# Sovik-Ghosh/SFM

Hardware: AMD Instinct MI355X
Metric: BA LM-iterations/sec + descriptor-pairs/sec, 200 cams / 100k pts, 1->8 MI355X (higher is better)
Workload: dtype f64; 1 GPU; BA: 200 cams / 100000 pts / 1000000 obs, cam block 10 (reference 10-parameter block + regulariser), aligned residual order, Huber, SciPy-TRF control flow, fixed schedule; parallelism=points sharded over 1 rank(s), cameras replicated, RCCL all-reduce of [S|r], comm=single rank, seed=1004

## Files before the change

### sfm_amd/csrc/ba.hip

```cpp
#include "ba_internal.h"
#include <cstdlib>
#include <type_traits>
#include <cmath>
#include <atomic>
#include <chrono>

typedef double v4d __attribute__((ext_vector_type(4)));

__device__ __forceinline__ void publish_word(double* word, double seq) {
  if (seq > 0.0) {
    __threadfence_system();
    *(volatile double*)word = seq;
  }
}
__device__ __forceinline__ void publish_ticket(double* hsc, double seq) { publish_word(hsc + SFM_HSC_SEQ, seq); }

#define EPS_D 2.220446049250313e-16
#define SQRT_EPS_D 1.4901161193847656e-08
#define CAMPRE 16

static int64_t g_stride(int64_t D) { return D == 10 ? 32 : 3 * D; }

Lay ba_layout(int64_t C, int64_t P, int64_t N, int64_t D, int64_t n_items, int64_t n_cchunks, int precision) {
  Lay L;
// ... 916 lines not shown
  }
  __syncthreads();
  if (Einv && r < c_0 + ASM_NB && e < D)
    diag_block_factor_lanes<D>(&sOut[0][(r - c_0) * D], ASM_NB * D + 1, alpha, e, r, Einv, Efac, cg_scal);
  const int n = C * D, W = nv * D;
  constexpr int WMAX = ASM_NB * D, NST = (D * WMAX + 127) / 128;
#pragma unroll
  for (int t = 0; t < NST; ++t) {
    const int idx = e + 128 * t;
    const int rr = idx / WMAX, col = idx - rr * WMAX;
    if (rr < D && col < W) S[(size_t)(r * D + rr) * n + c_0 * D + col] = sOut[rr][col];
  }
}

template <int D>
__global__ __launch_bounds__(128) void k_schur_diag(int C, const int* __restrict__ item_ptr, const double* __restrict__ part,
                                                    const double* __restrict__ B, double alpha, double* __restrict__ Einv,
                                                    double* __restrict__ Efac, double* __restrict__ cg_scal) {
  __shared__ double sBlk[D][D + 1];
  const int r = blockIdx.x, e = threadIdx.x;
  if (e < D * D) {
    const int rr = e / D, col = e - rr * D;
    const int64_t blk = (int64_t)r * C - (int64_t)r * (r - 1) / 2;
    double s = 0.0;
#pragma unroll 4
    for (int it = item_ptr[blk]; it < item_ptr[blk + 1]; ++it) s += part[(size_t)it * (D * D) + e];
    double v = -s;
    v += B[(size_t)r * D * D + e];
    sBlk[rr][col] = v;
  }
  __syncthreads();
  if (e < D) diag_block_factor_lanes<D>(&sBlk[0][0], D + 1, alpha, e, r, Einv, Efac, cg_scal);
}
template <int D, int ASM_NB>
__global__ __launch_bounds__(128) void k_schur_assemble_scaled(int C, const int* __restrict__ item_ptr, const double* __restrict__ part,
                                                               const double* __restrict__ B, double* __restrict__ St,
                                                               const int* __restrict__ cch_ptr, const double* __restrict__ cch_part,
                                                               const double* __restrict__ gc, double* __restrict__ rhs_out,
                                                               double* __restrict__ rhs_t, double alpha, const double* __restrict__ Einv) {
  constexpr int SCALED_BAND = 128 / D + 2;
  if (blockIdx.y == 0 && threadIdx.x < 64) {
    const int cc = blockIdx.x, lane = threadIdx.x, sl = lane >> 4, a = lane & 15;
    double t = 0.0;
    for (int ch = cch_ptr[cc] + sl; ch < cch_ptr[cc + 1]; ch += 4) t += cch_part[(size_t)ch * 16 + a];
    const double t1 = __shfl(t, a + 16, 64), t2 = __shfl(t, a + 32, 64), t3 = __shfl(t, a + 48, 64);
    const double rv = (sl == 0 && a < D) ? gc[cc * D + a] - ((t + t1) + (t2 + t3)) : 0.0;
    double ts = 0.0;
#pragma unroll
    for (int k = 0; k < D; ++k) ts += Einv[(size_t)cc * D * D + (a < D ? a : 0) * D + k] * __shfl(rv, k, 64);
    if (sl == 0 && a < D) { rhs_out[cc * D + a] = rv; rhs_t[cc * D + a] = ts; }
  }
  __shared__ double sOut[D][ASM_NB * D + 1];
  __shared__ double sE1[D * D], sE2[ASM_NB][D * D];
  const int r = blockIdx.x, c_0 = blockIdx.y * ASM_NB;
  if (c_0 > r) return;
  const int nv = (r - c_0 + 1) < ASM_NB ? (r - c_0 + 1) : ASM_NB;
  const int e = threadIdx.x;
  const int a = e / D, b = e - a * D;
  if (e < D * D) {
    double ev[ASM_NB + 1];
    ev[ASM_NB] = Einv[(size_t)r * D * D + e];
#pragma unroll
    for (int j = 0; j < ASM_NB; ++j) ev[j] = j < nv ? Einv[(size_t)(c_0 + j) * D * D + e] : 0.0;
    double v[ASM_NB];
    strip_item_sums<D, ASM_NB>(C, r, c_0, nv, e, item_ptr, part, B, v);
    sE1[e] = ev[ASM_NB];
#pragma unroll
    for (int j = 0; j < ASM_NB; ++j)
      if (j < nv) { sOut[a][j * D + b] = v[j]; sE2[j][e] = ev[j]; }
  }
  __syncthreads();
  const bool has_diag = r < c_0 + ASM_NB;
  const int jd = (r - c_0) * D;
  double dv = 0.0;
  if (has_diag && e < D * D) dv = (b <= a ? sOut[a][jd + b] : sOut[b][jd + a]) + (a == b ? alpha : 0.0);
  __syncthreads();
  if (has_diag && e < D * D) sOut[a][jd + b] = dv;
  __syncthreads();
  constexpr int RPT = 1;
  constexpr int RH = D / RPT;
  const int oj = e / RH, oh = e - oj * RH;
  const bool owner = e < ASM_NB * RH && oj < nv;
  double out[RPT][D];
  if (owner) {
#pragma unroll
    for (int q = 0; q < RPT; ++q) {
      const int ra = oh + q * RH;
      double tr[D];
#pragma unroll
      for (int bb = 0; bb < D; ++bb) tr[bb] = 0.0;
#pragma unroll
      for (int k = 0; k < D; ++k) {
        const double e1 = sE1[ra * D + k];
#pragma unroll
        for (int bb = 0; bb < D; ++bb) tr[bb] = fma(e1, sOut[k][oj * D + bb], tr[bb]);
        __builtin_amdgcn_sched_barrier(0);
      }
#pragma unroll
      for (int bb = 0; bb < D; ++bb) {
        double t = 0.0;
#pragma unroll
        for (int k = 0; k < D; ++k) t = fma(tr[k], sE2[oj][bb * D + k], t);
        out[q][bb] = t;
        __builtin_amdgcn_sched_barrier(0);
      }
    }
  }
  __syncthreads();
  if (owner) {
#pragma unroll
    for (int q = 0; q < RPT; ++q)
#pragma unroll
      for (int bb = 0; bb < D; ++bb) sOut[oh + q * RH][oj * D + bb] = out[q][bb];
  }
  __syncthreads();
  const int n = C * D, W = nv * D;
  constexpr int WMAX = ASM_NB * D, NST = (D * WMAX + 127) / 128;
#pragma unroll
  for (int t = 0; t < NST; ++t) {
    const int idx = e + 128 * t;
    const int rr = idx / WMAX, col = idx - rr * WMAX;
    if (rr < D && col < W) St[(size_t)(r * D + rr) * n + c_0 * D + col] = sOut[rr][col];
  }
  if (e < D * D) {
#pragma unroll
    for (int j = 0; j < ASM_NB; ++j) {
      const int c = c_0 + j;
      if (j < nv && c < r && r - c <= SCALED_BAND)
        St[(size_t)(c * D + a) * n + r * D + b] = sOut[b][j * D + a];
    }
  }
}

template <int D, typename T, int GS>
__global__ __launch_bounds__(256) void k_cam_reduce_chunks(const int* __restrict__ cch_beg, const int* __restrict__ cch_end,
                                                           const int* __restrict__ cam_obs, const int* __restrict__ cam_pt,
                                                           const T* __restrict__ G, const double* __restrict__ vec,
                                                           double* __restrict__ part) {
  static_assert(D % 2 == 0 && GS % 2 == 0 && GS <= 32, "16-byte pieces of a block: one per lane of a 16-lane group");
  typedef T pair_t __attribute__((ext_vector_type(2)));
  __shared__ double s[4][4][32];
  const int ch = blockIdx.x, tid = threadIdx.x, lane = tid & 63, w = tid >> 6;
  const int grp = lane >> 4, l16 = lane & 15;
  const int e0 = 2 * l16;
  const bool live = e0 < 3 * D;
  const int m = live ? e0 / D : 0;
  double acc0 = 0.0, acc1 = 0.0;
  const int beg = cch_beg[ch], end = cch_end[ch];
  constexpr int UNR = 4;
  for (int i0 = beg + w * 4 + grp; i0 < end; i0 += 16 * UNR) {
// ... 1 lines not shown
    pair_t g[UNR];
    double vm[UNR];
#pragma unroll
    for (int u = 0; u < UNR; ++u) { const int i = i0 + 16 * u; k[u] = i < end ? cam_obs[i] : -1; pj[u] = i < end ? cam_pt[i] : 0; }
#pragma unroll
    for (int u = 0; u < UNR; ++u) {
      g[u] = (k[u] >= 0 && live) ? *(const pair_t*)(G + (size_t)k[u] * GS + e0) : (pair_t){(T)0, (T)0};
    }
#pragma unroll
    for (int u = 0; u < UNR; ++u) vm[u] = k[u] >= 0 ? vec[(size_t)pj[u] * 3 + m] : 0.0;
#pragma unroll
    for (int u = 0; u < UNR; ++u)
      if (k[u] >= 0 && live) { acc0 += (double)g[u].x * vm[u]; acc1 += (double)g[u].y * vm[u]; }
  }
  s[w][grp][e0] = acc0; s[w][grp][e0 + 1] = acc1;
  __syncthreads();
  if (tid < 16) {
    double t = 0.0;
    if (tid < D) {
#pragma unroll
      for (int mm = 0; mm < 3; ++mm)
#pragma unroll
        for (int ww = 0; ww < 4; ++ww)
#pragma unroll
          for (int gg = 0; gg < 4; ++gg) t += s[ww][gg][mm * D + tid];
    }
    part[(size_t)ch * 16 + tid] = t;
  }
}
template <int D>
__global__ __launch_bounds__(256) void k_cam_reduce_final(int C, const int* __restrict__ cch_ptr, const double* __restrict__ part,
                                                          const double* __restrict__ base, double* __restrict__ out,
                                                          const double* __restrict__ sum_part = nullptr, int sum_nblk = 0, int sum_cnt = 0,
                                                          double* __restrict__ sum_dst = nullptr) {
  if (sum_part && blockIdx.x == gridDim.x - 1) {
    __shared__ double s_red[4];
    for (int q = 0; q < sum_cnt; ++q) {
      double t = 0.0;
      for (int i = threadIdx.x; i < sum_nblk; i += 256) t += sum_part[(size_t)i * sum_cnt + q];
      const double tt = block_sum256(t, s_red);
      if (threadIdx.x == 0) sum_dst[q] = tt;
    }
    return;
  }
  const int c = blockIdx.x * 4 + (threadIdx.x >> 6);
  if (c >= C) return;
  const int lane = threadIdx.x & 63, s = lane >> 4, a = lane & 15;
  double t = 0.0;
  for (int ch = cch_ptr[c] + s; ch < cch_ptr[c + 1]; ch += 4) t += part[(size_t)ch * 16 + a];
  const double t1 = __shfl(t, a + 16, 64), t2 = __shfl(t, a + 32, 64), t3 = __shfl(t, a + 48, 64);
  if (s == 0 && a < D) out[c * D + a] = (base ? base[c * D + a] : 0.0) - ((t + t1) + (t2 + t3));
}

constexpr int GTP_OBS = 64;
template <int D, typename T, int GS>
__global__ __launch_bounds__(256) void k_obs_Gtp(int64_t N, const int* __restrict__ cam_idx,
                                                 const T* __restrict__ G,
                                                 const double* __restrict__ pc, double* __restrict__ tmp3) {
  static_assert(D % 2 == 0 && GS % 2 == 0 && GS <= 32, "16-byte pieces of a block: one per lane of a 16-lane group");
  typedef T pair_t __attribute__((ext_vector_type(2)));
  __shared__ double s[GTP_OBS][17];
  const int tid = threadIdx.x, slot = tid >> 4, l16 = tid & 15;
  const int64_t k0 = (int64_t)blockIdx.x * GTP_OBS;
  const int e0 = 2 * l16;
  const int a = e0 % D;
  const bool live = e0 < 3 * D;
  pair_t g[GTP_OBS / 16];
  int cam[GTP_OBS / 16];
#pragma unroll
  for (int it = 0; it < GTP_OBS / 16; ++it) {
    const int64_t k = k0 + it * 16 + slot;
    const bool ok = live && k < N;
    g[it] = ok ? *(const pair_t*)(G + (size_t)k * GS + e0) : (pair_t)(T)0;
    cam[it] = ok ? cam_idx[k] : 0;
  }
#pragma unroll
  for (int it = 0; it < GTP_OBS / 16; ++it) {
    const double2 p = *(const double2*)(pc + (size_t)cam[it] * D + a);
    s[it * 16 + slot][l16] = (double)g[it].x * p.x + (double)g[it].y * p.y;
  }
  __syncthreads();
  if (tid < 3 * GTP_OBS) {
    const int sl = tid / 3, mm = tid - 3 * sl;
    const int64_t kk = k0 + sl;
// ... 383 lines not shown
  }
  hipLaunchKernelGGL(k_lin_finalize, dim3(1), dim3(256), 0, h->stream, n, D, WS(L, gc), WS(L, B), WS(L, part_obs),
                     (int)L.nblk_obs, WS(L, part_pt), (int)L.nblk_pt, WS(L, cost_reg), nreg, WS(L, red_lin),
                     WS(L, gmax));
  sfm_prof_end(h, SFM_PROF_LIN_REST);
  SFM_LAUNCH_CHECK(h, "sfm_ba_linearize");
  return SFM_OK;
}

extern "C" int sfm_ba_finish_linearize(sfm_handle h, sfm_ba_problem p) {
  Lay L; int rc = check_problem(h, p, &L); if (rc) return rc;
  double* ws = (double*)p->workspace;
  hipLaunchKernelGGL(k_finish_linearize, dim3(1), dim3(256), 0, h->stream, p->n_cams * p->cam_dim,
                     WS(L, red_lin), WS(L, gmax), WS(L, scalars), p->host_sc, next_ticket(p));
  SFM_LAUNCH_CHECK(h, "sfm_ba_finish_linearize");
  return SFM_OK;
}

static void launch_schur_assemble(sfm_ctx* h, sfm_ba_problem p, const Lay& L, double alpha, double* einv_out, double* m_out) {
  double* ws = (double*)p->workspace;
  const int C = p->n_cams, D = p->cam_dim, n = C * D;
  const AsmShape shape = schur_assemble_shape(C);
#define ASM_LAUNCH(NB, ROUNDS)                                                                                                  \
  hipLaunchKernelGGL((k_schur_assemble<DD, NB, ROUNDS>), dim3(C, cdiv(C, NB)), dim3(128), 0, h->stream, C, p->item_ptr,          \
                     WS(L, sch_part), WS(L, B), WS(L, red_S), WS(L, cg_scal), p->cch_ptr, WS(L, cch_part), WS(L, gc),             \
                     WS(L, red_S) + (size_t)n * n, alpha, einv_out, m_out)
  DISPATCH_D(D, {
    if (shape.rounds) ASM_LAUNCH(8, true);
    else if (shape.nb == 8) ASM_LAUNCH(8, false);
    else ASM_LAUNCH(2, false);
  });
#undef ASM_LAUNCH
}
static void launch_schur_assemble_scaled(sfm_ctx* h, sfm_ba_problem p, const Lay& L, double alpha, double* St) {
  double* ws = (double*)p->workspace;
  const int C = p->n_cams, D = p->cam_dim, n = C * D;
#define ASM_LAUNCH(NB)                                                                                                          \
  hipLaunchKernelGGL((k_schur_assemble_scaled<DD, NB>), dim3(C, cdiv(C, NB)), dim3(128), 0, h->stream, C, p->item_ptr,           \
                     WS(L, sch_part), WS(L, B), St, p->cch_ptr, WS(L, cch_part), WS(L, gc), WS(L, red_S) + (size_t)n * n,         \
                     WS(L, cg_r), alpha, WS(L, cg_Minv))
  DISPATCH_D(D, {
    hipLaunchKernelGGL(k_schur_diag<DD>, dim3(C), dim3(128), 0, h->stream, C, p->item_ptr, WS(L, sch_part), WS(L, B), alpha,
                       WS(L, cg_Minv), WS(L, cg_M), WS(L, cg_scal));
    if (schur_assemble_scaled_nb(C) == 4) ASM_LAUNCH(4);
    else ASM_LAUNCH(2);
  });
#undef ASM_LAUNCH
}

extern "C" int sfm_ba_schur_build(sfm_handle h, sfm_ba_problem p, double alpha) {
  Lay L; int rc = check_problem(h, p, &L); if (rc) return rc;
  if (!(alpha > 0.0)) return sfm_fail(h, SFM_ERR_ARG, "sfm_ba_schur_build", "alpha must be > 0");
  double* ws = (double*)p->workspace;
  const int C = p->n_cams, P = p->n_pts, D = p->cam_dim, n = C * D;
  const int64_t N = p->n_obs;
  const BaSwitches sw = ba_switches_from_env();
  const CamPlan plan = cam_plan(n, p->camera_solver, h->cgs_persist_off != 0, sw);
  sfm_prof_begin(h, SFM_PROF_BUILD_G);
  DISPATCH_DT(D, p->precision, {
    hipLaunchKernelGGL((k_build_G<DD, TT, double, GG>), dim3(cdiv(N, 256) + cdiv(P, 256)), dim3(256), 0, h->stream, N, p->pt_idx, WST(L, recA),
                       WST(L, recB), WS(L, Linv), WS(L, G), WS(L, e), WS(L, eobs), WS(L, Cp), WS(L, gp), alpha, P, (unsigned)cdiv(N, 256),
                       WS(L, cg_scal));
    sfm_prof_end(h, SFM_PROF_BUILD_G);
    sfm_prof_begin(h, SFM_PROF_SCHUR);
    if (p->n_items > 0) {
      sfm_prof_begin(h, SFM_PROF_SCHUR_ITEMS);
      hipLaunchKernelGGL((k_schur_items<DD, double, GG>), dim3(8 * cdiv(p->xcd_max_items, SFM_SCHUR_WG_WAVES)),
                         dim3(64 * SFM_SCHUR_WG_WAVES), 0, h->stream,
                         p->xcd_ptr, p->xcd_items, p->item_beg, p->item_end, p->pair_k, p->pair_k2, WS(L, G), WS(L, sch_part),
                         p->cam_idx, p->item_ptr, p->cch_ptr, C, WS(L, eobs), WS(L, cch_part), p->has_dup ? 0 : 1);
      sfm_prof_end(h, SFM_PROF_SCHUR_ITEMS);
    }
    if (p->has_dup && p->n_cchunks > 0)
      hipLaunchKernelGGL((k_cam_reduce_chunks<DD, double, GG>), dim3((unsigned)p->n_cchunks), dim3(256), 0, h->stream, p->cch_beg,
                         p->cch_end, p->cam_obs, p->cam_pt, WS(L, G), WS(L, e), WS(L, cch_part));
  });
  const BuildFusion fuse = build_fusion(plan, p->sharded != 0, p->camera_solver, n, sw);
  p->st_alpha = -1.0;
  p->s_valid = fuse.scale ? 0 : 1;
  if (fuse.scale) {
    DenseWs dw; dense_ws_carve(WS(L, dense), n, &dw);
    launch_schur_assemble_scaled(h, p, L, alpha, dw.Lm);
    p->st_alpha = alpha;
  } else
    launch_schur_assemble(h, p, L, alpha, fuse.einv ? WS(L, cg_Minv) : (double*)nullptr, WS(L, cg_M));
  p->cg_scal_clean = 1;
  p->einv_alpha = fuse.einv ? alpha : -1.0;
  sfm_prof_end(h, SFM_PROF_SCHUR);
  SFM_LAUNCH_CHECK(h, "sfm_ba_schur_build");
  return SFM_OK;
}

static int schur_materialise_S(sfm_ctx* h, sfm_ba_problem p, const Lay& L) {
  if (p->s_valid) return SFM_OK;
  launch_schur_assemble(h, p, L, 0.0, nullptr, nullptr);
  p->s_valid = 1;
  SFM_LAUNCH_CHECK(h, "schur_materialise_S");
  return SFM_OK;
}

__global__ __launch_bounds__(256) void k_pack_lower(const double* __restrict__ S, int n, double* __restrict__ Sp, int unpack_dir) {
  const int r = blockIdx.x;
  const int len = r < n ? r + 1 : n;
  const size_t off = (size_t)r * (r + 1) / 2;
  double* full = const_cast<double*>(S) + (size_t)r * n;
  for (int c = threadIdx.x; c < len; c += 256) {
    if (unpack_dir) full[c] = Sp[off + c];
    else Sp[off + c] = full[c];
  }
}

static int pack_S(sfm_handle h, sfm_ba_problem p, int unpack_dir, const char* what) {
  Lay L; int rc = check_problem(h, p, &L); if (rc) return rc;
  double* ws = (double*)p->workspace;
  const int n = p->n_cams * p->cam_dim;
// ... 836 lines not shown
    if (hst[CGS_FAIL] != 0.0) break;
    const double rr = hst[CGS_RR], rr0 = hst[CGS_RR0];
    const double done_its = hst[CGS_ITER] > 1.0 ? hst[CGS_ITER] : 1.0;
    const double rate = rr0 > 0.0 ? std::log(rr / rr0) / done_its : 0.0;
    batch = 8;
    if (rate < -1e-3 && rr > 0.0) {
      const double need = std::log(rtol2 * rr0 / rr) / rate;
      batch = need < 2.0 ? 3 : (need > 48.0 ? 48 : (int)need + 3);
    }
  }
  *iters_out += (int)hst[CGS_ITER];
  SFM_LAUNCH_CHECK(h, "cgs_solve_big");
  return SFM_OK;
}

static int cgs_solve_per_launch(sfm_ctx* h, sfm_ba_problem p, const Lay& L, const DenseWs& dw, const CamPlan& plan, int* status, int its_hint) {
  double* ws = (double*)p->workspace;
  const int n = p->n_cams * p->cam_dim;
  if (plan.per_launch == CAM_CG_TILES)
    return cgs_solve_big(h, n, dw.Lm, WS(L, cg_r), WS(L, cg_z), dw.LmT, WS(L, cg_scal), CGS_RTOL, plan.budget, &p->cg_iters, status, its_hint);
  return cgs_solve(h, n, dw.Lm, WS(L, cg_r), WS(L, cg_z), dw.LmT, WS(L, cg_scal), CGS_RTOL, &p->cg_iters, status);
}

static int factor_system(sfm_ctx* h, sfm_ba_problem p, const Lay& L, const DenseWs& dw, double alpha) {
  double* ws = (double*)p->workspace;
  const int n = p->n_cams * p->cam_dim;
  int rc = schur_materialise_S(h, p, L); if (rc) return rc;
  p->st_alpha = -1.0;
  SFM_HIP(h, hipMemsetAsync(dw.flag, 0, sizeof(int), h->stream));
  hipLaunchKernelGGL(k_add_diag, dim3(cdiv(n, 256)), dim3(256), 0, h->stream, WS(L, red_S), n, alpha);
  return dense_cholesky(h, WS(L, red_S), n, n + 1, dw);
}

static void launch_backsub(sfm_ctx* h, sfm_ba_problem p, const Lay& L, double* ws, int want_q) {
  const int C = p->n_cams, P = p->n_pts, D = p->cam_dim, n = C * D;
  const int64_t N = p->n_obs;
  sfm_prof_begin(h, SFM_PROF_BACKSUB);
  DISPATCH_DT(D, p->precision, hipLaunchKernelGGL((k_obs_Gtp<DD, double, GG>), dim3(cdiv(N, GTP_OBS)), dim3(256), 0, h->stream, N,
                                                  p->cam_idx, WS(L, G), WS(L, pc), WS(L, tmp3)));
  hipLaunchKernelGGL(k_backsub, dim3((unsigned)L.nblk_pt), dim3(256), 0, h->stream, P, p->pt_ptr, WS(L, tmp3),
                     WS(L, Linv), WS(L, e), WS(L, pp), WS(L, v), WS(L, part_pt));
  if (want_q) {
    DISPATCH_DT(D, p->precision, {
      if (p->n_cchunks > 0)
        hipLaunchKernelGGL((k_cam_reduce_chunks<DD, double, GG>), dim3((unsigned)p->n_cchunks), dim3(256), 0, h->stream, p->cch_beg,
                           p->cch_end, p->cam_obs, p->cam_pt, WS(L, G), WS(L, v), WS(L, cch_part));
      hipLaunchKernelGGL(k_cam_reduce_final<DD>, dim3(cdiv(C, 4) + 1), dim3(256), 0, h->stream, C, p->cch_ptr,
                         WS(L, cch_part), (const double*)nullptr, WS(L, red_q), WS(L, part_pt), (int)L.nblk_pt, 2, WS(L, red_q) + n);
    });
  } else {
    hipLaunchKernelGGL(k_sum_partials, dim3(1), dim3(256), 0, h->stream, WS(L, part_pt), (int)L.nblk_pt, 2,
                       WS(L, red_q) + n);
  }
  sfm_prof_end(h, SFM_PROF_BACKSUB);
}

extern "C" int sfm_ba_set_sharded(sfm_handle h, sfm_ba_problem p, int sharded) {
  if (!h) return SFM_ERR_ARG;
  if (!p) return sfm_fail(h, SFM_ERR_ARG, "sfm_ba_set_sharded", "null problem");
  p->sharded = sharded ? 1 : 0;
  return SFM_OK;
}

extern "C" int sfm_ba_schur_solve(sfm_handle h, sfm_ba_problem p, double alpha, int want_q) {
  Lay L; int rc = check_problem(h, p, &L); if (rc) return rc;
  double* ws = (double*)p->workspace;
  const int C = p->n_cams, D = p->cam_dim, n = C * D;
  double* S = WS(L, red_S);
  DenseWs dw; dense_ws_carve(WS(L, dense), n, &dw);
  p->cg_state = 0;
  p->cg2_pending = 0;
  p->cg_alpha = alpha;
  const BaSwitches sw = ba_switches_from_env();
  const CamPlan plan = cam_plan(n, p->camera_solver, h->cgs_persist_off != 0, sw);
  const double hdiag = p->host_sc[SFM_SC_HDIAG];
  const double arel = hdiag > 0.0 ? alpha / hdiag : 0.0;
  const bool hopeless = p->camera_solver == SFM_CAMERA_SOLVER_AUTO && arel > 0.0 && sw.predict && p->cgp.hopeless(arel, plan.budget);
  if (hopeless) p->cg_fallbacks++;
  if (plan.route != CAM_FACTOR && !hopeless) {
    const int its_before = p->cg_iters;
    sfm_prof_begin(h, SFM_PROF_CHOL);
    if (!p->cg_scal_clean) { SFM_HIP(h, hipMemsetAsync(WS(L, cg_scal), 0, CG_SCAL_WORDS * sizeof(double), h->stream)); p->einv_alpha = -1.0; }
    p->cg_scal_clean = 0;
    const bool have_einv = p->einv_alpha == alpha && !p->sharded;
    p->einv_alpha = -1.0;
    const bool have_st = have_einv && p->st_alpha == alpha && plan.lower_only;
    if (!have_st && (rc = schur_materialise_S(h, p, L))) return rc;
    if (!have_st) DISPATCH_D(D, {
      if (!have_einv)
        hipLaunchKernelGGL(k_diag_einv<DD>, dim3(cdiv(C, 64)), dim3(64), 0, h->stream, C, S, n, alpha, WS(L, cg_Minv), WS(L, cg_M), WS(L, cg_scal));
      if (plan.lower_only)
        hipLaunchKernelGGL(k_scale_system_lower<DD>, dim3(C, cdiv(C, SCALE_NB)), dim3(128), 0, h->stream, n, C, S, alpha, WS(L, cg_Minv), dw.Lm,
                           S + (size_t)n * n, WS(L, cg_r));
      else
        hipLaunchKernelGGL(k_scale_system<DD>, dim3(C, cdiv(C, SCALE_NB)), dim3(128), 0, h->stream, n, C, S, alpha, WS(L, cg_Minv), dw.Lm,
                           S + (size_t)n * n, WS(L, cg_r));
    });
    int status = 1, ran = 0;
    if (plan.route == CAM_CG_PERSIST) {
      PrFuse fuse = {WS(L, cg_Minv), nullptr, WS(L, pc), nullptr, nullptr, nullptr, nullptr, 1, 0.0};
      const PrLaunch pl = {n, D, dw.Lm, WS(L, cg_r), WS(L, cg_z), WS(L, cg_mail), WS(L, cg_scal), CGS_RTOL, fuse, h->pinned + SFM_PIN_CG1};
      rc = cgs_persist_launch(h, pl);
      if (rc) return rc;
      SFM_HIP(h, hipEventRecord(h->cg_event, h->stream));
      sfm_prof_end(h, SFM_PROF_CHOL);
      launch_backsub(h, p, L, ws, want_q);
      SFM_HIP(h, hipEventSynchronize(h->cg_event));
      int relaunched = 0;
      rc = cgs_persist_verdict(h, pl, p->sharded, &p->cg_iters, &status, &ran, &relaunched);
      if (rc) return rc;
      if (relaunched && ran && status == 0) launch_backsub(h, p, L, ws, want_q);
      if (ran && status == 0) {
        p->cg_state = 1;
        p->cgp.note_ok(arel, p->cg_iters - its_before);
        SFM_LAUNCH_CHECK(h, "sfm_ba_schur_solve");
        return SFM_OK;
      }
      sfm_prof_begin(h, SFM_PROF_CHOL);
    }
    if (!ran) {
      DISPATCH_D(D, hipLaunchKernelGGL(k_block_mv<DD>, dim3(cdiv(n, 256)), dim3(256), 0, h->stream, C, WS(L, cg_Minv), S + (size_t)n * n, WS(L, cg_r), 0, 1.0));
      rc = cgs_solve_per_launch(h, p, L, dw, plan, &status, p->cgp.ok_its[0]);
      if (rc) return rc;
      p->cg_its_sys1 = p->cg_iters - its_before;
      if (status == 0)
        DISPATCH_D(D, hipLaunchKernelGGL(k_block_mv<DD>, dim3(cdiv(n, 256)), dim3(256), 0, h->stream, C, WS(L, cg_Minv), WS(L, cg_z),
                                         WS(L, pc), 1, -1.0));
    }
    if (status == 0) {
      p->cg_state = 1;
      p->cgp.note_ok(arel, p->cg_iters - its_before);
    } else {
      p->cg_fallbacks++;
      p->cgp.note_out_of_budget(arel, p->cg_iters - its_before, plan.budget);
    }
    sfm_prof_end(h, SFM_PROF_CHOL);
  }
  if (p->cg_state == 0) {
    sfm_prof_begin(h, SFM_PROF_CHOL);
    rc = factor_system(h, p, L, dw, alpha); if (rc) return rc;
    sfm_prof_end(h, SFM_PROF_CHOL);
    sfm_prof_begin(h, SFM_PROF_TRSV);
    hipLaunchKernelGGL(k_copy_neg, dim3(cdiv(n, 256)), dim3(256), 0, h->stream, dw.Lm + (size_t)n * n, WS(L, tvec), n, -1.0);
    rc = dense_trsv(h, n, dw, WS(L, tvec), WS(L, pc), 1); if (rc) return rc;
// ... 7 lines not shown
static int finish_solve_by_factor(sfm_ctx* h, sfm_ba_problem p, const Lay& L, double* ws, int want_q, bool factor_first) {
  const int n = p->n_cams * p->cam_dim;
  DenseWs dw; dense_ws_carve(WS(L, dense), n, &dw);
  int rc;
  if (factor_first) {
    p->cg_fallbacks++;
    p->cg_state = 0;
    rc = factor_system(h, p, L, dw, p->cg_alpha); if (rc) return rc;
  }
  if (want_q) {
    sfm_prof_begin(h, SFM_PROF_TRSV);
    hipLaunchKernelGGL(k_add_vec, dim3(cdiv(n, 256)), dim3(256), 0, h->stream, WS(L, pc), WS(L, red_q), WS(L, tvec), n);
    rc = dense_trsv(h, n, dw, WS(L, tvec), WS(L, y), 0); if (rc) return rc;
    sfm_prof_end(h, SFM_PROF_TRSV);
  }
  hipLaunchKernelGGL(k_finish_solve, dim3(1), dim3(256), 0, h->stream, n, WS(L, pc), WS(L, red_q), WS(L, y),
                     want_q, (const int*)dw.flag, WS(L, scalars), p->host_sc, next_ticket(p));
  SFM_LAUNCH_CHECK(h, "sfm_ba_finish_solve");
  return SFM_OK;
}

extern "C" int sfm_ba_finish_solve(sfm_handle h, sfm_ba_problem p, int want_q) {
  Lay L; int rc = check_problem(h, p, &L); if (rc) return rc;
  double* ws = (double*)p->workspace;
  const int n = p->n_cams * p->cam_dim;
  DenseWs dw; dense_ws_carve(WS(L, dense), n, &dw);
  const CamPlan plan = cam_plan(n, p->camera_solver, h->cgs_persist_off != 0, ba_switches_from_env());
  if (p->cg_state == 1) {
    const int C = p->n_cams, D = p->cam_dim;
    int status = 0;
    if (want_q) {
      sfm_prof_begin(h, SFM_PROF_TRSV);
      if (plan.route == CAM_CG_PERSIST) {
        DISPATCH_D(D, hipLaunchKernelGGL(k_block_mv<DD>, dim3(cdiv(n, 256)), dim3(256), 0, h->stream, C, WS(L, cg_Minv), WS(L, pc),
                                         WS(L, cg_r), 0, 1.0, WS(L, red_q)));
        PrFuse fuse = {WS(L, cg_Minv), nullptr, nullptr, WS(L, pc), WS(L, red_q), WS(L, scalars), p->host_sc, 1, next_ticket(p)};
        const PrLaunch pl = {n, D, dw.Lm, WS(L, cg_r), WS(L, cg_z), WS(L, cg_mail), WS(L, cg_scal), CGS_RTOL, fuse, p->host_sc + SFM_HSC_CG2};
        rc = cgs_persist_launch(h, pl);
        if (rc) return rc;
        p->cg2_pending = 1;
        sfm_prof_end(h, SFM_PROF_TRSV);
        return SFM_OK;
      }
      hipLaunchKernelGGL(k_add_vec, dim3(cdiv(n, 256)), dim3(256), 0, h->stream, WS(L, pc), WS(L, red_q), WS(L, tvec), n);
      DISPATCH_D(D, hipLaunchKernelGGL(k_block_mv<DD>, dim3(cdiv(n, 256)), dim3(256), 0, h->stream, C, WS(L, cg_Minv), WS(L, tvec),
                                       WS(L, cg_r), 0, 1.0));
      rc = cgs_solve_per_launch(h, p, L, dw, plan, &status, p->cg_its_sys1);
      if (rc) return rc;
      if (status == 0)
        hipLaunchKernelGGL(k_dot, dim3(1), dim3(1024), 0, h->stream, n, WS(L, cg_r), WS(L, cg_z), WS(L, cg_scal) + 8);
      sfm_prof_end(h, SFM_PROF_TRSV);
    }
    if (status == 0) {
      hipLaunchKernelGGL(k_finish_solve_pcg, dim3(1), dim3(256), 0, h->stream, n, WS(L, pc), WS(L, red_q), want_q, WS(L, cg_scal) + 8,
                         WS(L, cg_scal) + CGS_FAIL, WS(L, scalars), p->host_sc, next_ticket(p));
      SFM_LAUNCH_CHECK(h, "sfm_ba_finish_solve");
      return SFM_OK;
    }
    return finish_solve_by_factor(h, p, L, ws, want_q, true);
  }
  return finish_solve_by_factor(h, p, L, ws, want_q, false);
}

enum { CG_RZ = 0, CG_RR = 1, CG_RR0 = 2, CG_ITER = 3, CG_FAIL = 4, CG_DOT = 5 };

__global__ __launch_bounds__(256) void k_track_sum(int P, const int* __restrict__ pt_ptr, const double* __restrict__ tmp3,
                                                   double* __restrict__ u) {
  const int j = blockIdx.x * 256 + threadIdx.x;
// ... 419 lines not shown
```

### sfm_amd/csrc/ba_internal.h

```cpp
#pragma once
#include "dense.h"
#include "ba_plan.h"

struct Lay {
  int64_t recA, recB, campre, campre2, B, gc, Cp, gp, Linv, e, v, tmp3, G, eobs, red_lin, gmax, red_S, red_q,
      red_step, pc, pp, y, tvec, scalars, part_obs, part_pt, part_x, cost_reg, regrec, dense, sch_part, cch_part, cbl_part,
      cg_r, cg_z, cg_p, cg_Ap, cg_M, cg_Minv, cg_scal, cg_mail, total;
  int64_t nblk_obs, nblk_pt;
};
constexpr int CG_SCAL_WORDS = 16;

struct sfm_ba_prob {
  sfm_ctx* h;
  int32_t n_cams, n_pts, cam_dim, apply_reg, precision;
  int64_t n_obs;
  double fx0, fy0, cx0, cy0, width, height, reg_weight;
  int32_t *cam_idx, *pt_idx;
  double* uv;
  int32_t *pt_ptr, *cam_ptr, *cam_obs, *blk_ptr, *pair_k, *pair_k2;
  int32_t* cam_pt;

  int64_t n_pairs;
  int32_t *item_ptr, *item_beg, *item_end;
  int64_t n_items;
  int32_t *xcd_ptr, *xcd_items;
  int64_t xcd_max_items;
  int32_t *cch_ptr, *cch_beg, *cch_end;
  int64_t n_cchunks;
  void* workspace;
  int64_t workspace_bytes;
  int owns_workspace;
  Lay L;
  int camera_solver, cg_state, cg_iters, cg_fallbacks;
  int cg2_pending;
  double* host_sc;
  double look_seq;
  int look_pending;
  int sharded;
  int cg_scal_clean;
  double einv_alpha;
  double st_alpha;
  int s_valid;
  int has_dup;
  int64_t pcg_fallbacks;
  double pcg_worst_relres;
  double cg_alpha;
  CgPredictor cgp;
  int cg_its_sys1;
};

constexpr int SFM_HSC_CG2 = SFM_SC_COUNT, SFM_HSC_SEQ = SFM_SC_COUNT + 8, SFM_HSC_WORDS = SFM_SC_COUNT + 16;

static inline double next_ticket(sfm_ba_prob* p) { p->look_seq += 1.0; p->look_pending = 1; return p->look_seq; }

Lay ba_layout(int64_t C, int64_t P, int64_t N, int64_t D, int64_t n_items, int64_t n_cchunks, int precision);

void* sfm_scratch(sfm_ctx* h, size_t bytes);

int ba_xnorm_partial(sfm_ctx* h, sfm_ba_problem p, const double* x);
int ba_xnorm_finish(sfm_ctx* h, sfm_ba_problem p, const double* x);
```

### sfm_amd/csrc/ba_plan.h

```cpp
#pragma once
#include <cmath>
#include <cstdint>
#include <cstdlib>

#ifdef SFM_BA_PLAN_STANDALONE
enum { SFM_CAMERA_SOLVER_AUTO = 0, SFM_CAMERA_SOLVER_CHOLESKY = 1, SFM_CAMERA_SOLVER_CG = 2 };
#endif

constexpr int PR_MAX_N = 2048;
constexpr int CGS_MAX_N = 4096;
constexpr int CGS_MAX_ITER = 160;
constexpr int CGS_BIG_MAX_ITER = 400;
constexpr int ASM_ROUNDS_FROM = 512;
constexpr int ASM_WIDE_FROM = 128;

struct BaSwitches {
  bool persist;
  bool big;
  int big_from;
  int big_budget;
  bool predict;
  bool fuse_scale;
};
static inline bool ba_switch_on(const char* name) { const char* e = getenv(name); return !(e && e[0] == '0'); }
static inline BaSwitches ba_switches_from_env() {
  BaSwitches s;
  s.persist = ba_switch_on("SFM_CGS_PERSIST");
  s.big = ba_switch_on("SFM_CGS_BIG");
  const char* f = getenv("SFM_CGS_BIG_FROM");
  s.big_from = f ? (atoi(f) > 256 ? atoi(f) : 257) : PR_MAX_N + 1;
  const char* b = getenv("SFM_CGS_BIG_BUDGET");
  const int v = b ? atoi(b) : 0;
  s.big_budget = v > 0 ? v : CGS_BIG_MAX_ITER;
  s.predict = ba_switch_on("SFM_CGS_PREDICT");
  s.fuse_scale = ba_switch_on("SFM_SCHUR_FUSE_SCALE");
  return s;
}

enum CamRoute {
  CAM_FACTOR,
  CAM_CG_PERSIST,
  CAM_CG_ITER,
  CAM_CG_TILES
};
struct CamPlan {
  CamRoute route;
  CamRoute per_launch;
  bool lower_only;
  int budget;
};
static inline CamPlan cam_plan(int n, int camera_solver, bool persist_off, const BaSwitches& sw) {
  const bool even = (n & 1) == 0;
  const bool big = sw.big && n >= sw.big_from;
  CamPlan pl;
  pl.per_launch = big ? CAM_CG_TILES : CAM_CG_ITER;
  pl.budget = big ? sw.big_budget : CGS_MAX_ITER;
  if (camera_solver == SFM_CAMERA_SOLVER_CHOLESKY || !even || (n > CGS_MAX_N && !big)) pl.route = CAM_FACTOR;
  else if (n <= PR_MAX_N && !persist_off && sw.persist) pl.route = CAM_CG_PERSIST;
  else pl.route = pl.per_launch;
  pl.lower_only = pl.route == CAM_CG_TILES;
  return pl;
}

struct BuildFusion {
  bool einv;
  bool scale;
};
static inline BuildFusion build_fusion(const CamPlan& plan, bool sharded, int camera_solver, int n, const BaSwitches& sw) {
  BuildFusion f;
  f.einv = !sharded && camera_solver != SFM_CAMERA_SOLVER_CHOLESKY && (n & 1) == 0;
  f.scale = sw.fuse_scale && f.einv && plan.lower_only;
  return f;
}

struct AsmShape { int nb; bool rounds; };
static inline AsmShape schur_assemble_shape(int C) {
  if (C >= ASM_ROUNDS_FROM) return {8, true};
  if (C >= ASM_WIDE_FROM) return {8, false};
  return {2, false};
}
static inline int schur_assemble_scaled_nb(int C) { return C >= ASM_WIDE_FROM ? 4 : 2; }

struct CgPredictor {
  double fail_rel, ok_rel[2];
  int ok_its[2];

  bool hopeless(double arel, int budget) const {
    if (fail_rel > 0.0 && arel <= 4.0 * fail_rel) return true;
    if (ok_its[0] > 0 && arel < ok_rel[0]) {
      double slope = 0.2;
      if (ok_its[1] > 0) {
        slope = -std::log((double)ok_its[0] / ok_its[1]) / std::log(ok_rel[0] / ok_rel[1]);
        slope = slope < 0.0 ? 0.0 : (slope > 0.5 ? 0.5 : slope);
      }
      if (ok_its[0] * std::pow(ok_rel[0] / arel, 0.85 * slope) > 1.25 * budget) return true;
    }
    return false;
  }
  void note_ok(double arel, int its) {
    if (its <= 0) return;
    if (ok_its[0] > 0) {
      const double r = arel / ok_rel[0];
      if (r >= 1.5 || r <= 1.0 / 1.5) { ok_rel[1] = ok_rel[0]; ok_its[1] = ok_its[0]; }
    }
// ... 8 lines not shown
```

### sfm_amd/csrc/problem.hip

```cpp
#include <cstdlib>
#include <cstring>
#include <vector>
#include "ba_internal.h"
#include <rocprim/device/device_radix_sort.hpp>
#include <rocprim/device/device_scan.hpp>

#define ITEM_PAIRS 256
#define CHUNK_OBS 256

namespace {

__global__ __launch_bounds__(256) void k_tracks(int64_t N, int P, int C, const int* __restrict__ cam_idx,
                                                const int* __restrict__ pt_idx, int* __restrict__ pt_ptr,
                                                int* __restrict__ cam_cnt, int* __restrict__ err) {
  const int64_t k = (int64_t)blockIdx.x * 256 + threadIdx.x;
  if (k >= N) return;
  const int c = cam_idx[k], j = pt_idx[k];
  const int prev = k > 0 ? pt_idx[k - 1] : -1;
  const bool ok = c >= 0 && c < C && j >= 0 && j < P && prev >= -1 && prev < P;
  if (!ok) { atomicOr(err, 1); return; }
  if (prev > j) { atomicOr(err, 2); return; }
  atomicAdd(&cam_cnt[c], 1);
  for (int q = prev + 1; q <= j; ++q) pt_ptr[q] = (int)k;
  if (k == N - 1)
// ... 136 lines not shown
  void* owned[] = {p->cam_idx, p->pt_idx, p->uv, p->pt_ptr, p->cam_ptr, p->cam_obs, p->cam_pt, p->blk_ptr, p->pair_k, p->pair_k2,
                   p->item_ptr, p->item_beg, p->item_end, p->xcd_ptr, p->xcd_items, p->cch_ptr, p->cch_beg, p->cch_end};
  for (void* q : owned)
    if (q) (void)hipFree(q);
  if (p->owns_workspace && p->workspace) (void)hipFree(p->workspace);
  if (p->host_sc) (void)hipHostFree(p->host_sc);
  delete p;
}

extern "C" int sfm_ba_create_problem(sfm_handle h, const sfm_ba_desc* d, sfm_ba_problem* out) {
  if (!h) return SFM_ERR_ARG;
  if (!d || !out) return sfm_fail(h, SFM_ERR_ARG, "sfm_ba_create_problem", "null argument");
  if (d->n_cams < 1 || d->n_pts < 1 || d->n_obs < 1 || (d->cam_dim != 6 && d->cam_dim != 10))
    return sfm_fail(h, SFM_ERR_ARG, "sfm_ba_create_problem", "bad problem sizes / cam_dim");
  if (!d->cam_idx || !d->pt_idx || !d->uv) return sfm_fail(h, SFM_ERR_ARG, "sfm_ba_create_problem", "null index / pixel array");
  if ((int64_t)d->n_cams * d->cam_dim > 32000) return sfm_fail(h, SFM_ERR_ARG, "sfm_ba_create_problem", "reduced system too large");
  if (d->n_obs >= (1ll << 31)) return sfm_fail(h, SFM_ERR_ARG, "sfm_ba_create_problem", "too many observations for int32 indices");
  if (d->precision != SFM_BA_FP64 && d->precision != SFM_BA_MIXED)
    return sfm_fail(h, SFM_ERR_ARG, "sfm_ba_create_problem", "unknown precision");
  if (d->camera_solver < SFM_CAMERA_SOLVER_AUTO || d->camera_solver > SFM_CAMERA_SOLVER_CG)
    return sfm_fail(h, SFM_ERR_ARG, "sfm_ba_create_problem", "unknown camera_solver");
  if (d->uv_pairing != SFM_UV_AS_GIVEN && d->uv_pairing != SFM_UV_REFERENCE_PAIRING)
    return sfm_fail(h, SFM_ERR_ARG, "sfm_ba_create_problem", "unknown uv_pairing");
  const int C = d->n_cams, P = d->n_pts;
  const int64_t N = d->n_obs;
  const int64_t n_blk = (int64_t)C * (C + 1) / 2;
  hipStream_t st = h->stream;

  sfm_ba_prob* p = new sfm_ba_prob();
  memset(p, 0, sizeof(*p));
  p->h = h;
  p->n_cams = C; p->n_pts = P; p->cam_dim = d->cam_dim; p->apply_reg = d->apply_reg; p->precision = d->precision;
  p->camera_solver = d->camera_solver;
  p->einv_alpha = -1.0; p->st_alpha = -1.0; p->s_valid = 1;
  if (hipHostMalloc((void**)&p->host_sc, SFM_HSC_WORDS * sizeof(double), hipHostMallocDefault) != hipSuccess) {
    p->host_sc = nullptr; sfm_ba_destroy_problem(p);
    return sfm_fail(h, SFM_ERR_HIP, "sfm_ba_create_problem", "pinned host memory for the scalars");
  }
  memset(p->host_sc, 0, SFM_HSC_WORDS * sizeof(double));
  p->n_obs = N;
  p->fx0 = d->fx0; p->fy0 = d->fy0; p->cx0 = d->cx0; p->cy0 = d->cy0;
  p->width = d->width; p->height = d->height; p->reg_weight = d->reg_weight;

  PB_HIP(hipMalloc((void**)&p->cam_idx, N * 4));
  PB_HIP(hipMalloc((void**)&p->pt_idx, N * 4));
  PB_HIP(hipMalloc((void**)&p->uv, N * 16));
  PB_HIP(hipMemcpyAsync(p->cam_idx, d->cam_idx, N * 4, hipMemcpyDefault, st));
  PB_HIP(hipMemcpyAsync(p->pt_idx, d->pt_idx, N * 4, hipMemcpyDefault, st));
  PB_HIP(hipMemcpyAsync(p->uv, d->uv, N * 16, hipMemcpyDefault, st));

  PB_HIP(hipMalloc((void**)&p->pt_ptr, ((int64_t)P + 1) * 4));
  PB_HIP(hipMalloc((void**)&p->cam_ptr, ((int64_t)C + 1) * 4));
  DevBuf small;
  PB_HIP(small.alloc(((int64_t)4 * C + 8) * 4));
  int* cam_cnt = small.as<int>();
  int* err = cam_cnt + C;
  int* row_first = err + 1;
  int* row_cnt = row_first + C;
  int* row_base = row_cnt + C;
  PB_HIP(hipMemsetAsync(cam_cnt, 0, ((int64_t)C + 1) * 4, st));
  PB_HIP(hipMemsetAsync(p->pt_ptr, 0, ((int64_t)P + 1) * 4, st));
  hipLaunchKernelGGL(k_tracks, dim3(cdiv(N, 256)), dim3(256), 0, st, N, P, C, p->cam_idx, p->pt_idx, p->pt_ptr, cam_cnt, err);
  hipLaunchKernelGGL(k_scan_small, dim3(1), dim3(1), 0, st, cam_cnt, C, p->cam_ptr);
  {
    int herr = 0;
    PB_HIP(hipMemcpyAsync(&herr, err, 4, hipMemcpyDeviceToHost, st));
    PB_HIP(hipStreamSynchronize(st));
// ... 210 lines not shown
```

Before: 246.4 LM-iterations/s.

## Fuse full scaled Schur assembly and second preconditioned residual into existing kernels

Extends the scaled Schur assembly kernel with a FULL variant that also writes the unscaled S and fills the full upper triangle of the scaled matrix, so the persistent-CG route can reuse it instead of materialising S in a separate pass. It also fuses the block-diagonal preconditioner multiply for the second solve into the camera reduce-final kernel, skipping a separate k_block_mv launch. The cost is extra register and global-store traffic in the assembly kernel, plus more per-solve state flags (st_full, rt2_ready) that must stay consistent.

```diff
diff --git a/sfm_amd/csrc/ba.hip b/sfm_amd/csrc/ba.hip
--- a/sfm_amd/csrc/ba.hip
+++ b/sfm_amd/csrc/ba.hip
@@ -972,13 +972,14 @@
   __syncthreads();
   if (e < D) diag_block_factor_lanes<D>(&sBlk[0][0], D + 1, alpha, e, r, Einv, Efac, cg_scal);
 }
-template <int D, int ASM_NB>
+template <int D, int ASM_NB, bool FULL>
 __global__ __launch_bounds__(128) void k_schur_assemble_scaled(int C, const int* __restrict__ item_ptr, const double* __restrict__ part,
                                                                const double* __restrict__ B, double* __restrict__ St,
                                                                const int* __restrict__ cch_ptr, const double* __restrict__ cch_part,
                                                                const double* __restrict__ gc, double* __restrict__ rhs_out,
-                                                               double* __restrict__ rhs_t, double alpha, const double* __restrict__ Einv) {
-  constexpr int SCALED_BAND = 128 / D + 2;
+                                                               double* __restrict__ rhs_t, double alpha, const double* __restrict__ Einv,
+                                                               double* __restrict__ S_out ) {
+  constexpr int SCALED_BAND = FULL ? (1 << 30) : 128 / D + 2;
   if (blockIdx.y == 0 && threadIdx.x < 64) {
     const int cc = blockIdx.x, lane = threadIdx.x, sl = lane >> 4, a = lane & 15;
     double t = 0.0;
@@ -1012,6 +1013,16 @@
   __syncthreads();
   const bool has_diag = r < c_0 + ASM_NB;
   const int jd = (r - c_0) * D;
+  const int n = C * D, W = nv * D;
+  constexpr int WMAX = ASM_NB * D, NST = (D * WMAX + 127) / 128;
+  if (FULL) {
+#pragma unroll
+    for (int t = 0; t < NST; ++t) {
+      const int idx = e + 128 * t;
+      const int rr = idx / WMAX, col = idx - rr * WMAX;
+      if (rr < D && col < W) S_out[(size_t)(r * D + rr) * n + c_0 * D + col] = sOut[rr][col];
+    }
+  }
   double dv = 0.0;
   if (has_diag && e < D * D) dv = (b <= a ? sOut[a][jd + b] : sOut[b][jd + a]) + (a == b ? alpha : 0.0);
   __syncthreads();
@@ -1021,8 +1032,30 @@
   constexpr int RH = D / RPT;
   const int oj = e / RH, oh = e - oj * RH;
   const bool owner = e < ASM_NB * RH && oj < nv;
+  const bool upper_form = FULL && c_0 + oj != r;
+  static_assert(!FULL || RPT == 1, "the upper form is written for one row per thread");
   double out[RPT][D];
-  if (owner) {
+  if (FULL && owner && upper_form) {
+    double tr[D];
+#pragma unroll
+    for (int bb = 0; bb < D; ++bb) tr[bb] = 0.0;
+#pragma unroll
+    for (int k = 0; k < D; ++k) {
+      const double e2 = sE2[oj][oh * D + k];
+#pragma unroll
+      for (int bb = 0; bb < D; ++bb) tr[bb] = fma(e2, sOut[bb][oj * D + k], tr[bb]);
+      __builtin_amdgcn_sched_barrier(0);
+    }
+#pragma unroll
+    for (int bb = 0; bb < D; ++bb) {
+      double t = 0.0;
+#pragma unroll
+      for (int k = 0; k < D; ++k) t = fma(tr[k], sE1[bb * D + k], t);
+      out[0][bb] = t;
+      __builtin_amdgcn_sched_barrier(0);
+    }
+  }
+  if (owner && !upper_form) {
 #pragma unroll
     for (int q = 0; q < RPT; ++q) {
       const int ra = oh + q * RH;
@@ -1051,11 +1084,12 @@
 #pragma unroll
     for (int q = 0; q < RPT; ++q)
 #pragma unroll
-      for (int bb = 0; bb < D; ++bb) sOut[oh + q * RH][oj * D + bb] = out[q][bb];
-  }
-  __syncthreads();
-  const int n = C * D, W = nv * D;
-  constexpr int WMAX = ASM_NB * D, NST = (D * WMAX + 127) / 128;
+      for (int bb = 0; bb < D; ++bb) {
+        if (upper_form) sOut[bb][oj * D + oh] = out[q][bb];
+        else sOut[oh + q * RH][oj * D + bb] = out[q][bb];
+      }
+  }
+  __syncthreads();
 #pragma unroll
   for (int t = 0; t < NST; ++t) {
     const int idx = e + 128 * t;
@@ -1123,7 +1157,9 @@
 __global__ __launch_bounds__(256) void k_cam_reduce_final(int C, const int* __restrict__ cch_ptr, const double* __restrict__ part,
                                                           const double* __restrict__ base, double* __restrict__ out,
                                                           const double* __restrict__ sum_part = nullptr, int sum_nblk = 0, int sum_cnt = 0,
-                                                          double* __restrict__ sum_dst = nullptr) {
+                                                          double* __restrict__ sum_dst = nullptr,
+                                                          const double* __restrict__ rt_add = nullptr, const double* __restrict__ rt_Einv = nullptr,
+                                                          double* __restrict__ rt_out = nullptr) {
   if (sum_part && blockIdx.x == gridDim.x - 1) {
     __shared__ double s_red[4];
     for (int q = 0; q < sum_cnt; ++q) {
@@ -1140,7 +1176,17 @@
   double t = 0.0;
   for (int ch = cch_ptr[c] + s; ch < cch_ptr[c + 1]; ch += 4) t += part[(size_t)ch * 16 + a];
   const double t1 = __shfl(t, a + 16, 64), t2 = __shfl(t, a + 32, 64), t3 = __shfl(t, a + 48, 64);
-  if (s == 0 && a < D) out[c * D + a] = (base ? base[c * D + a] : 0.0) - ((t + t1) + (t2 + t3));
+  const bool mine = s == 0 && a < D;
+  const double o = mine ? (base ? base[c * D + a] : 0.0) - ((t + t1) + (t2 + t3)) : 0.0;
+  if (mine) out[c * D + a] = o;
+  if (rt_out) {
+    const double v = mine ? rt_add[c * D + a] + o : 0.0;
+    const double* E = rt_Einv + (size_t)c * D * D + (a < D ? a : 0) * D;
+    double ts = 0.0;
+#pragma unroll
+    for (int k = 0; k < D; ++k) ts += E[k] * __shfl(v, k, 64);
+    if (mine) rt_out[c * D + a] = ts;
+  }
 }
 
 constexpr int GTP_OBS = 64;
@@ -1590,18 +1636,18 @@
   });
 #undef ASM_LAUNCH
 }
-static void launch_schur_assemble_scaled(sfm_ctx* h, sfm_ba_problem p, const Lay& L, double alpha, double* St) {
+static void launch_schur_assemble_scaled(sfm_ctx* h, sfm_ba_problem p, const Lay& L, double alpha, double* St, bool full) {
   double* ws = (double*)p->workspace;
   const int C = p->n_cams, D = p->cam_dim, n = C * D;
-#define ASM_LAUNCH(NB)                                                                                                          \
-  hipLaunchKernelGGL((k_schur_assemble_scaled<DD, NB>), dim3(C, cdiv(C, NB)), dim3(128), 0, h->stream, C, p->item_ptr,           \
+#define ASM_LAUNCH(NB, FULL)                                                                                                    \
+  hipLaunchKernelGGL((k_schur_assemble_scaled<DD, NB, FULL>), dim3(C, cdiv(C, NB)), dim3(128), 0, h->stream, C, p->item_ptr,     \
                      WS(L, sch_part), WS(L, B), St, p->cch_ptr, WS(L, cch_part), WS(L, gc), WS(L, red_S) + (size_t)n * n,         \
-                     WS(L, cg_r), alpha, WS(L, cg_Minv))
+                     WS(L, cg_r), alpha, WS(L, cg_Minv), WS(L, red_S))
   DISPATCH_D(D, {
     hipLaunchKernelGGL(k_schur_diag<DD>, dim3(C), dim3(128), 0, h->stream, C, p->item_ptr, WS(L, sch_part), WS(L, B), alpha,
                        WS(L, cg_Minv), WS(L, cg_M), WS(L, cg_scal));
-    if (schur_assemble_scaled_nb(C) == 4) ASM_LAUNCH(4);
-    else ASM_LAUNCH(2);
+    if (schur_assemble_scaled_nb(C) == 4) { if (full) ASM_LAUNCH(4, true); else ASM_LAUNCH(4, false); }
+    else { if (full) ASM_LAUNCH(2, true); else ASM_LAUNCH(2, false); }
   });
 #undef ASM_LAUNCH
 }
@@ -1636,9 +1682,10 @@
   const BuildFusion fuse = build_fusion(plan, p->sharded != 0, p->camera_solver, n, sw);
   p->st_alpha = -1.0;
   p->s_valid = fuse.scale ? 0 : 1;
-  if (fuse.scale) {
+  p->st_full = fuse.scale_full ? 1 : 0;
+  if (fuse.scale || fuse.scale_full) {
     DenseWs dw; dense_ws_carve(WS(L, dense), n, &dw);
-    launch_schur_assemble_scaled(h, p, L, alpha, dw.Lm);
+    launch_schur_assemble_scaled(h, p, L, alpha, dw.Lm, fuse.scale_full);
     p->st_alpha = alpha;
   } else
     launch_schur_assemble(h, p, L, alpha, fuse.einv ? WS(L, cg_Minv) : (double*)nullptr, WS(L, cg_M));
@@ -2541,7 +2588,7 @@
   return dense_cholesky(h, WS(L, red_S), n, n + 1, dw);
 }
 
-static void launch_backsub(sfm_ctx* h, sfm_ba_problem p, const Lay& L, double* ws, int want_q) {
+static void launch_backsub(sfm_ctx* h, sfm_ba_problem p, const Lay& L, double* ws, int want_q, bool rt2 = false) {
   const int C = p->n_cams, P = p->n_pts, D = p->cam_dim, n = C * D;
   const int64_t N = p->n_obs;
   sfm_prof_begin(h, SFM_PROF_BACKSUB);
@@ -2555,8 +2602,11 @@
         hipLaunchKernelGGL((k_cam_reduce_chunks<DD, double, GG>), dim3((unsigned)p->n_cchunks), dim3(256), 0, h->stream, p->cch_beg,
                            p->cch_end, p->cam_obs, p->cam_pt, WS(L, G), WS(L, v), WS(L, cch_part));
       hipLaunchKernelGGL(k_cam_reduce_final<DD>, dim3(cdiv(C, 4) + 1), dim3(256), 0, h->stream, C, p->cch_ptr,
-                         WS(L, cch_part), (const double*)nullptr, WS(L, red_q), WS(L, part_pt), (int)L.nblk_pt, 2, WS(L, red_q) + n);
+                         WS(L, cch_part), (const double*)nullptr, WS(L, red_q), WS(L, part_pt), (int)L.nblk_pt, 2, WS(L, red_q) + n,
+                         rt2 ? WS(L, pc) : (const double*)nullptr, rt2 ? WS(L, cg_Minv) : (const double*)nullptr,
+                         rt2 ? WS(L, cg_r) : (double*)nullptr);
     });
+    p->rt2_ready = rt2 ? 1 : 0;
   } else {
     hipLaunchKernelGGL(k_sum_partials, dim3(1), dim3(256), 0, h->stream, WS(L, part_pt), (int)L.nblk_pt, 2,
                        WS(L, red_q) + n);
@@ -2579,6 +2629,7 @@
   DenseWs dw; dense_ws_carve(WS(L, dense), n, &dw);
   p->cg_state = 0;
   p->cg2_pending = 0;
+  p->rt2_ready = 0;
   p->cg_alpha = alpha;
   const BaSwitches sw = ba_switches_from_env();
   const CamPlan plan = cam_plan(n, p->camera_solver, h->cgs_persist_off != 0, sw);
@@ -2593,7 +2644,7 @@
     p->cg_scal_clean = 0;
     const bool have_einv = p->einv_alpha == alpha && !p->sharded;
     p->einv_alpha = -1.0;
-    const bool have_st = have_einv && p->st_alpha == alpha && plan.lower_only;
+    const bool have_st = have_einv && p->st_alpha == alpha && (p->st_full || plan.lower_only);
     if (!have_st && (rc = schur_materialise_S(h, p, L))) return rc;
     if (!have_st) DISPATCH_D(D, {
       if (!have_einv)
@@ -2613,12 +2664,13 @@
       if (rc) return rc;
       SFM_HIP(h, hipEventRecord(h->cg_event, h->stream));
       sfm_prof_end(h, SFM_PROF_CHOL);
-      launch_backsub(h, p, L, ws, want_q);
+      const bool rt2 = !p->sharded;
+      launch_backsub(h, p, L, ws, want_q, rt2);
       SFM_HIP(h, hipEventSynchronize(h->cg_event));
       int relaunched = 0;
       rc = cgs_persist_verdict(h, pl, p->sharded, &p->cg_iters, &status, &ran, &relaunched);
       if (rc) return rc;
-      if (relaunched && ran && status == 0) launch_backsub(h, p, L, ws, want_q);
+      if (relaunched && ran && status == 0) launch_backsub(h, p, L, ws, want_q, rt2);
       if (ran && status == 0) {
         p->cg_state = 1;
         p->cgp.note_ok(arel, p->cg_iters - its_before);
@@ -2692,8 +2744,10 @@
     if (want_q) {
       sfm_prof_begin(h, SFM_PROF_TRSV);
       if (plan.route == CAM_CG_PERSIST) {
-        DISPATCH_D(D, hipLaunchKernelGGL(k_block_mv<DD>, dim3(cdiv(n, 256)), dim3(256), 0, h->stream, C, WS(L, cg_Minv), WS(L, pc),
-                                         WS(L, cg_r), 0, 1.0, WS(L, red_q)));
+        if (!p->rt2_ready)
+          DISPATCH_D(D, hipLaunchKernelGGL(k_block_mv<DD>, dim3(cdiv(n, 256)), dim3(256), 0, h->stream, C, WS(L, cg_Minv), WS(L, pc),
+                                           WS(L, cg_r), 0, 1.0, WS(L, red_q)));
+        p->rt2_ready = 0;
         PrFuse fuse = {WS(L, cg_Minv), nullptr, nullptr, WS(L, pc), WS(L, red_q), WS(L, scalars), p->host_sc, 1, next_ticket(p)};
         const PrLaunch pl = {n, D, dw.Lm, WS(L, cg_r), WS(L, cg_z), WS(L, cg_mail), WS(L, cg_scal), CGS_RTOL, fuse, p->host_sc + SFM_HSC_CG2};
         rc = cgs_persist_launch(h, pl);
diff --git a/sfm_amd/csrc/ba_internal.h b/sfm_amd/csrc/ba_internal.h
--- a/sfm_amd/csrc/ba_internal.h
+++ b/sfm_amd/csrc/ba_internal.h
@@ -33,6 +33,7 @@
   Lay L;
   int camera_solver, cg_state, cg_iters, cg_fallbacks;
   int cg2_pending;
+  int rt2_ready;
   double* host_sc;
   double look_seq;
   int look_pending;
@@ -40,6 +41,7 @@
   int cg_scal_clean;
   double einv_alpha;
   double st_alpha;
+  int st_full;
   int s_valid;
   int has_dup;
   int64_t pcg_fallbacks;
diff --git a/sfm_amd/csrc/ba_plan.h b/sfm_amd/csrc/ba_plan.h
--- a/sfm_amd/csrc/ba_plan.h
+++ b/sfm_amd/csrc/ba_plan.h
@@ -47,6 +47,7 @@
   CamRoute route;
   CamRoute per_launch;
   bool lower_only;
+  bool st_from_tiles;
   int budget;
 };
 static inline CamPlan cam_plan(int n, int camera_solver, bool persist_off, const BaSwitches& sw) {
@@ -59,17 +60,20 @@
   else if (n <= PR_MAX_N && !persist_off && sw.persist) pl.route = CAM_CG_PERSIST;
   else pl.route = pl.per_launch;
   pl.lower_only = pl.route == CAM_CG_TILES;
+  pl.st_from_tiles = pl.route == CAM_CG_PERSIST;
   return pl;
 }
 
 struct BuildFusion {
   bool einv;
   bool scale;
+  bool scale_full;
 };
 static inline BuildFusion build_fusion(const CamPlan& plan, bool sharded, int camera_solver, int n, const BaSwitches& sw) {
   BuildFusion f;
   f.einv = !sharded && camera_solver != SFM_CAMERA_SOLVER_CHOLESKY && (n & 1) == 0;
   f.scale = sw.fuse_scale && f.einv && plan.lower_only;
+  f.scale_full = sw.fuse_scale && f.einv && plan.st_from_tiles;
   return f;
 }
 
diff --git a/sfm_amd/csrc/problem.hip b/sfm_amd/csrc/problem.hip
--- a/sfm_amd/csrc/problem.hip
+++ b/sfm_amd/csrc/problem.hip
@@ -192,7 +192,7 @@
   p->h = h;
   p->n_cams = C; p->n_pts = P; p->cam_dim = d->cam_dim; p->apply_reg = d->apply_reg; p->precision = d->precision;
   p->camera_solver = d->camera_solver;
-  p->einv_alpha = -1.0; p->st_alpha = -1.0; p->s_valid = 1;
+  p->einv_alpha = -1.0; p->st_alpha = -1.0; p->s_valid = 1; p->st_full = 0; p->rt2_ready = 0;
   if (hipHostMalloc((void**)&p->host_sc, SFM_HSC_WORDS * sizeof(double), hipHostMallocDefault) != hipSuccess) {
     p->host_sc = nullptr; sfm_ba_destroy_problem(p);
     return sfm_fail(h, SFM_ERR_HIP, "sfm_ba_create_problem", "pinned host memory for the scalars");
```

After: 246.3 LM-iterations/s. About the same (-0.0%).
